# AdamBeedell/MLX8-WS-Audio-Transformer

Measured on AMD Instinct MI355X. Metric: 4s@16kHz clips/sec through mel+Whisper-small encoder, higher is better.
Workload: dtype fp16; 1 GPU; int16 PCM [B,64000] in HBM -> Whisper log-mel [B,80,3000] -> Whisper-small encoder -> hidden [B,1500,768] fp32; mode=parity (clip zero-padded to 30 s, as the reference computes), precision=f16f8, fp16_exact_projection_matrices=0 of 48 (found by the library at upload), parallelism=dp1 (clip shards, no data-path collective)

## Files before the change

### include/awt.h

```cpp
#ifndef AWT_H_
#define AWT_H_

#include <stddef.h>
#include <stdint.h>

#ifdef __cplusplus
extern "C" {
#endif

typedef enum awt_status {
  AWT_OK = 0,
  AWT_ERR_INVALID = -1,
  AWT_ERR_HIP = -2,
  AWT_ERR_WORKSPACE = -3,
  AWT_ERR_STATE = -4,
  AWT_ERR_VALUE = -5
} awt_status;

typedef struct awt_ctx awt_ctx;
typedef struct awt_encoder awt_encoder;

const char* awt_last_error(void);
const char* awt_version(void);

// ... 176 lines not shown
                            float* out, void* stream);
size_t awt_dtw_workspace_bytes(int clips, int T, int frames);
int awt_op_dtw(awt_ctx* c, const float* matrix, int clips, int T, int frames, const int32_t* num_frames, int negate, int32_t* jump_frame,
               int32_t* text_idx, int32_t* time_idx, int32_t* path_start, void* workspace, size_t ws_bytes, void* stream);

size_t awt_op_conv1d_workspace_bytes(int B, int T, int Cin, int Cout);
int awt_op_conv1d(awt_ctx* c, const float* x, const float* w, const float* bias, float* y, int B, int T, int Cin, int Cout, int taps, int terms,
                  void* workspace, size_t ws_bytes, void* stream);
size_t awt_op_batchnorm_stats_workspace_bytes(int M, int C);
int awt_op_batchnorm_stats(awt_ctx* c, const float* x, int M, int C, float* mean, float* var, void* workspace, size_t ws_bytes, void* stream);
enum { AWT_POOL_MEAN = 0, AWT_POOL_MAX2 = 2, AWT_POOL_MAX4 = 4, AWT_POOL_MAX4_MEAN = 5 };
int awt_op_bn_relu_pool(awt_ctx* c, const float* x, const float* mean, const float* var, const float* gamma, const float* beta, float eps,
                        float* y, int B, int T, int C, int pool, void* stream);
size_t awt_op_bn_relu_pool_backward_workspace_bytes(int B, int T, int C);
int awt_op_bn_relu_pool_backward(awt_ctx* c, const float* dy, const float* x, const float* mean, const float* var, const float* gamma,
                                 const float* beta, float eps, float* dx, float* dgamma, float* dbeta, int B, int T, int C, int pool,
                                 void* workspace, size_t ws_bytes, void* stream);

int awt_op_conv1d_framed(awt_ctx* c, const float* x, int64_t x_pitch, const float* w, const float* bias, float* y, int B, int n_samples, int kernel,
                         int stride, int Cout, void* stream);

int awt_tuning_set(const char* key, int value);

enum { AWT_PROF_LOGMEL = 0, AWT_PROF_GEMM = 1, AWT_PROF_ATTENTION = 2, AWT_PROF_LAYERNORM = 3, AWT_PROF_OTHER = 4,
       AWT_PROF_ATTENTION_BWD = 5,
       AWT_PROF_WGRAD = 6,
       AWT_PROF_NCLASSES = 7 };
int awt_prof_enable(awt_ctx* c, int mask);
int awt_prof_collect(awt_ctx* c, int klass, double* total_ms, int64_t* launches, double* flops);

#ifdef __cplusplus
}
#endif
#endif
```

### mlx8-ws-audio-transformer_amd/_lib.py

```python
from __future__ import annotations

import ctypes as C
import os
import re
import threading
from typing import Optional

import torch

HERE = os.path.dirname(os.path.abspath(__file__))
LIB_PATH = os.environ.get("AWT_LIB") or os.path.join(HERE, "libawt.so")
HEADER_PATH = os.path.join(os.path.dirname(HERE), "include", "awt.h")

AWT_OK = 0
AWT_ERR_VALUE = -5


class AwtError(RuntimeError):
    def __init__(self, code: int, msg: str):
        super().__init__(f"libawt error {code}: {msg}")
        self.code = code
        self.msg = msg


# ... 88 lines not shown
    "awt_op_attention_small": (_i, [_vp, _vp, _i, _vp, _i, _vp, _i, _vp, _i, _vp, _i, _i, _i, _i, _i, _i, _vp]),
    "awt_op_attention_small_backward": (_i, [_vp, _vp, _i, _vp, _i, _vp, _i, _vp, _vp, _i, _vp, _vp, _vp, _vp, _vp, _i, _i, _i, _i, _i, _i, _vp]),
    "awt_op_attention_small_dropout": (_i, [_vp, _vp, _i, _vp, _i, _vp, _i, _vp, _i, _vp, _i, _i, _i, _i, _i, _i, C.c_float, C.c_uint64, _vp]),
    "awt_op_attention_small_backward_dropout": (_i, [_vp, _vp, _i, _vp, _i, _vp, _i, _vp, _vp, _i, _vp, _vp, _vp, _vp, _vp, _i, _i, _i, _i, _i, _i, C.c_float, C.c_uint64, _vp]),
    "awt_op_attention_cached": (_i, [_vp, _vp, _i, _vp, _vp, _i, _i64, _vp, _i, _i, _i, _i, _i, _vp]),
    "awt_select_tokens_workspace_bytes": (_sz, [_i, _i, _i]),
    "awt_op_select_tokens": (_i, [_vp, _vp, _i, _i, _i, _i, _vp, _vp, _i, _i, _vp, _vp, _vp, _vp, _sz, _vp]),
    "awt_select_tokens_ts_workspace_bytes": (_sz, [_i, _i, _i]),
    "awt_op_select_tokens_ts": (_i, [_vp, _vp, _i, _i, _i, _i, _vp, _vp, _i, _i, _vp, _vp, _vp, _vp, _vp, _sz, _vp]),
    "awt_op_kv_gather": (_i, [_vp, _vp, _vp, _vp, _i, _i, _i, _i, _i, _i, _vp]),
    "awt_op_alignment_weights": (_i, [_vp, _vp, _i, _i, _i, _i, _i, _vp, _i, _i, _vp, _i, _vp, _i, _i, _i, _vp, _i, _vp]),
    "awt_op_alignment_matrix": (_i, [_vp, _vp, _i, _i, _i, _i, _vp, _i, _vp, _vp]),
    "awt_dtw_workspace_bytes": (_sz, [_i, _i, _i]),
    "awt_op_dtw": (_i, [_vp, _vp, _i, _i, _i, _vp, _i, _vp, _vp, _vp, _vp, _vp, _sz, _vp]),
    "awt_op_conv1d_workspace_bytes": (_sz, [_i, _i, _i, _i]),
    "awt_op_conv1d": (_i, [_vp, _vp, _vp, _vp, _vp, _i, _i, _i, _i, _i, _i, _vp, _sz, _vp]),
    "awt_op_batchnorm_stats_workspace_bytes": (_sz, [_i, _i]),
    "awt_op_batchnorm_stats": (_i, [_vp, _vp, _i, _i, _vp, _vp, _vp, _sz, _vp]),
    "awt_op_bn_relu_pool": (_i, [_vp, _vp, _vp, _vp, _vp, _vp, _f, _vp, _i, _i, _i, _i, _vp]),
    "awt_op_bn_relu_pool_backward_workspace_bytes": (_sz, [_i, _i, _i]),
    "awt_op_bn_relu_pool_backward": (_i, [_vp, _vp, _vp, _vp, _vp, _vp, _vp, _f, _vp, _vp, _vp, _i, _i, _i, _i, _vp, _sz, _vp]),
    "awt_op_conv1d_framed": (_i, [_vp, _vp, _i64, _vp, _vp, _vp, _i, _i, _i, _i, _i, _vp]),
    "awt_tuning_set": (_i, [C.c_char_p, _i]),
    "awt_prof_enable": (_i, [_vp, _i]),
    "awt_prof_collect": (_i, [_vp, _i, C.POINTER(C.c_double), C.POINTER(_i64), C.POINTER(C.c_double)]),
}

_lib = None
_lock = threading.Lock()
_ctx = {}


def declared_symbols() -> list:
    text = open(HEADER_PATH).read()
    text = re.sub(r"/\*.*?\*/", "", text, flags=re.S)
    return sorted(set(re.findall(r"\b(awt_[a-z0-9_]+)\s*\(", text)))


def lib() -> C.CDLL:
    global _lib
    with _lock:
        if _lib is None:
            if not os.path.exists(LIB_PATH):
                raise ImportError(f"{LIB_PATH} is missing: run `python -m mlx8_ws_audio_transformer_amd.build` "
                                  "(there is no CPU fallback for this path)")
            l = C.CDLL(LIB_PATH)
# ... 69 lines not shown
```

### mlx8-ws-audio-transformer_amd/csrc/awt_api.hip

```cpp
#include <string.h>
#include <algorithm>
#include <string>
#include <vector>

#include "common.h"
#include "comm.h"
#include "wgrad.h"

static thread_local std::string g_err;
void awt_set_error(const std::string& msg) { g_err = msg; }
int awt_fail(int code, const std::string& msg) { g_err = msg; return code; }
extern "C" const char* awt_last_error(void) { return g_err.c_str(); }
extern "C" const char* awt_version(void) { return "awt 0.1 (gfx950)"; }

struct awt_prof_state {
  struct Span { hipEvent_t a, b; };
  std::vector<Span> spans[AWT_PROF_NCLASSES];
  std::vector<Span> pool;
  double flops[AWT_PROF_NCLASSES] = {};
  Span open[AWT_PROF_NCLASSES];
};

void awt_prof_begin(awt_ctx* c, int klass, hipStream_t s, double flops) {
  awt_prof_state* p = c->prof;
// ... 14 lines not shown
static int g_pp_mask = 12;
extern "C" int awt_tuning_set(const char* key, int value) {
  AWT_REQUIRE(key, AWT_ERR_INVALID, "tuning_set: null key");
  if (!strcmp(key, "gemm_tile")) {
    AWT_REQUIRE(value == 0 || value == 64 || value == 128 || value == 256, AWT_ERR_INVALID, "tuning_set: gemm_tile must be 0 (auto), 64, 128 or 256");
    awt_gemm_force_tile(value);
    return AWT_OK;
  }
  if (!strcmp(key, "gemm_gm")) {
    AWT_REQUIRE(value >= 0 && value <= 64, AWT_ERR_INVALID, "tuning_set: gemm_gm must be 0 (default) .. 64");
    awt_gemm_set_gm(value);
    return AWT_OK;
  }
  if (!strcmp(key, "gemm_pp")) {
    AWT_REQUIRE(value >= 0 && value <= 2, AWT_ERR_INVALID, "tuning_set: gemm_pp must be 0 (off), 1 (automatic, default) or 2 (wherever supported)");
    awt_gemm_set_pp_mode(value);
    return AWT_OK;
  }
  if (!strcmp(key, "gemm_pp_mask")) {
    AWT_REQUIRE(value >= 0 && value <= 15, AWT_ERR_INVALID, "tuning_set: gemm_pp_mask is a bit set 0 .. 15 (1 qkv, 2 out_proj, 4 fc1, 8 fc2; fc2 only together with fc1)");
    g_pp_mask = value;
    return AWT_OK;
  }
  if (!strcmp(key, "gemm_mfma16")) {
    AWT_REQUIRE(value == 0 || value == 1, AWT_ERR_INVALID, "tuning_set: gemm_mfma16 must be 1 (default: the f16f8 GEMM's 16 x 16 MFMA form where it applies) or 0 (32 x 32 only)");
    awt_gemm_set_mfma16(value);
    return AWT_OK;
  }
  if (!strcmp(key, "conv_live")) {
    AWT_REQUIRE(value == 0 || value == 1, AWT_ERR_INVALID, "tuning_set: conv_live must be 1 (default: the conv stem of awt_audio_encode computes the live positions only) or 0 (every position)");
    g_conv_live = value;
    return AWT_OK;
  }
  if (!strcmp(key, "attn_shape")) {
    AWT_REQUIRE(value == 0 || (value >= 4 && value <= 6), AWT_ERR_INVALID, "tuning_set: attn_shape must be 0 (auto), 4, 5 or 6");
    awt_attn_force_shape(value);
    return AWT_OK;
  }
  if (!strcmp(key, "attn_qt")) {
    AWT_REQUIRE(value >= 0 && value <= 2, AWT_ERR_INVALID, "tuning_set: attn_qt must be 0 (auto), 1 or 2");
    awt_attn_force_qt(value);
    return AWT_OK;
  }
  AWT_REQUIRE(false, AWT_ERR_INVALID, "tuning_set: unknown key");
}

extern "C" int awt_prof_enable(awt_ctx* c, int on) {
  AWT_REQUIRE(c, AWT_ERR_INVALID, "prof_enable: null ctx");
  if (!c->prof) c->prof = new awt_prof_state();
  c->prof_on = on;
  return AWT_OK;
}
extern "C" int awt_prof_collect(awt_ctx* c, int klass, double* total_ms, int64_t* launches, double* flops) {
  AWT_REQUIRE(c && c->prof && klass >= 0 && klass < AWT_PROF_NCLASSES, AWT_ERR_INVALID, "prof_collect: bad argument");
  awt_prof_state* p = c->prof;
  double ms = 0;
  for (auto& sp : p->spans[klass]) {
    AWT_HIP_CHECK(hipEventSynchronize(sp.b));
    float t = 0;
    AWT_HIP_CHECK(hipEventElapsedTime(&t, sp.a, sp.b));
    ms += t;
    p->pool.push_back(sp);
  }
  if (total_ms) *total_ms = ms;
  if (launches) *launches = (int64_t)p->spans[klass].size();
  if (flops) *flops = p->flops[klass];
  p->spans[klass].clear();
  p->flops[klass] = 0;
// ... 1150 lines not shown
```

### mlx8-ws-audio-transformer_amd/csrc/common.h

```cpp
#pragma once
#include <hip/hip_runtime.h>
#include <stdint.h>
#include <string>

#include "../../include/awt.h"

typedef unsigned short bf16_t;
typedef short bf16x8 __attribute__((ext_vector_type(8)));
typedef short bf16x4 __attribute__((ext_vector_type(4)));
typedef float f32x4 __attribute__((ext_vector_type(4)));
typedef float f32x16 __attribute__((ext_vector_type(16)));
typedef double f64x4 __attribute__((ext_vector_type(4)));

typedef _Float16 f16x8 __attribute__((ext_vector_type(8)));
typedef int i32x8 __attribute__((ext_vector_type(8)));
typedef int i32x2 __attribute__((ext_vector_type(2)));

#define AWT_WAVE 64

enum { PREC_BF16 = 1, PREC_F16 = 2, PREC_BF16X3 = 3, PREC_F16X3 = 4, PREC_F16F8 = 5 };
__host__ __device__ constexpr bool prec_known(int p) { return p >= PREC_BF16 && p <= PREC_F16F8; }
__host__ __device__ constexpr bool prec_is_f16(int p) { return p == PREC_F16 || p == PREC_F16X3 || p == PREC_F16F8; }
__host__ __device__ constexpr int prec_products(int p) { return (p == PREC_BF16 || p == PREC_F16) ? 1 : 3; }
constexpr int kF8Act = -2;
// ... 292 lines not shown
  uint8_t* hi8; uint8_t* lo8;
  char* ilv;
  bf16_t* hi2; bf16_t* lo2;
  const bf16_t* pre_hi; const bf16_t* pre_lo;
  const float* bias;
  const float* pos; int rows_pos;
  float scale;
  int n_valid;
  int S, H;
  int64_t plane_stride;
  int skip_v8;
  int m_pick;
};

int launch_gemm(awt_ctx* c, int M, int N, const GemmSeg* segs, int nseg, int prec, GemmEpilogue epi, const GemmOut& out,
                hipStream_t s);
bool gemm_pp_supported(int M, int N, int K, int epi);
int gemm_pp_slots();
int launch_gemm_pp(awt_ctx* c, int M, int N, const GemmSeg& seg, GemmEpilogue epi, const GemmOut& out, hipStream_t s);
size_t gemm_pp_weight_bytes(int N, int K);
int launch_pack_weight_pp(awt_ctx* c, const float* src, int N, int K, int row_off, char* dst, hipStream_t s);
int awt_gemm_pp_mode();
void awt_gemm_set_pp_mode(int v);
void awt_gemm_set_mfma16(int v);

int launch_layernorm(awt_ctx* c, const float* x, const float* gamma, const float* beta, int M, int d, float eps,
                     float* out_f32, const Act& out, int prec, hipStream_t s);
int launch_attention(awt_ctx* c, const bf16_t* q_hi, const bf16_t* q_lo, const bf16_t* k_hi, const bf16_t* k_lo,
                     const bf16_t* v_hi, const bf16_t* v_lo, bf16_t* o_hi, bf16_t* o_lo, float* o_f32, float* lse, int B, int H,
                     int S, int terms, hipStream_t s);
int launch_split_f32(awt_ctx* c, const float* x, int64_t n, float scale, bf16_t* hi, bf16_t* lo, hipStream_t s);
struct F8Planes { bf16_t* p16; uint8_t* hi8; uint8_t* lo8; };
int launch_split_planes(awt_ctx* c, const float* x, int64_t n, float scale, int prec, int f8_exp, bf16_t* p16, bf16_t* lo16, uint8_t* hi8,
                        uint8_t* lo8, hipStream_t s, char* ilv = nullptr);
int launch_attention_f16f8(awt_ctx* c, const F8Planes& q, const F8Planes& k, const F8Planes& v, const F8Planes& o, float* o_f32,
                           float* lse, int B, int H, int S, hipStream_t s, char* o_ilv = nullptr);
int launch_pack_weight(awt_ctx* c, const float* src, int N, int C, int taps, int64_t ld, int row_off, int col_off, float scale,
                       bf16_t* hi, bf16_t* lo, uint8_t* lo8, int prec, hipStream_t s, int* inexact = nullptr,
                       bf16_t* s16 = nullptr, uint8_t* s8 = nullptr);
int launch_im2col_conv1(awt_ctx* c, const float* mel, int B, int C, int T_mel, int T, int K_dst, const Act& out, int prec, hipStream_t s);
int launch_expand_conv_rows(awt_ctx* c, const float* g, const float* pos, int B, int S, int Sc, int d, float* x, hipStream_t s);
int conv_stem_positions(int n_ctx, int max_valid);

int logmel_whisper_impl(awt_ctx* c, const void* pcm, int pcm_is_i16, int64_t pcm_stride, const int32_t* n_valid,
                        int max_valid, int B, int n_frames_out, int n_mels, float* out, void* workspace, size_t ws_bytes, hipStream_t s,
                        int n_signal = 0);
// ... 28 lines not shown
```

### mlx8-ws-audio-transformer_amd/csrc/gemm.hip

```cpp
#include <algorithm>
#include <type_traits>
#include "common.h"
#include "gemm_pp.h"

#ifndef AWT_GEMM_GM
#define AWT_GEMM_GM 8
#endif

namespace {

int g_gm = AWT_GEMM_GM;
constexpr int kMaxSeg = 3;
typedef int i32x4_t __attribute__((ext_vector_type(4)));

struct GemmArgs {
  int M, N, nseg, tiles_m, tiles_n;
  int gm;
  GemmSeg seg[kMaxSeg];
  GemmOut out;
  const bf16_t* zeros;
  int64_t bs_a, bs_w, bs_o;
};

struct Cfg64 { static constexpr int WM = 2, WN = 2, TM = 2, TN = 4; };
// ... 904 lines not shown
template <int EPI>
int launch_f8s(GemmArgs a, hipStream_t s) {
  return launch_tiles<gemm_f8s_kernel<EPI>>(a, 128, 256, 256, 2 * (128 * 64 * 2 + 2 * 128 * 64), s);
}

template <int EPI, class CFG>
int launch_f8(GemmArgs a, hipStream_t s) {
  constexpr int BM = CFG::WM * CFG::TM * 32, BN = CFG::WN * CFG::TN * 32, NT = CFG::WM * CFG::WN * 64;
  constexpr int lds = 2 * (BM * 64 * 2 + 2 * BM * 64);
  if (a.nseg == 1 && a.seg[0].w_exact16) return launch_tiles<gemm_f8_kernel<EPI, CFG, false, true>>(a, BM, BN, NT, lds, s);
  if (a.nseg == 1) return launch_tiles<gemm_f8_kernel<EPI, CFG, false>>(a, BM, BN, NT, lds, s);
  return launch_tiles<gemm_f8_kernel<EPI, CFG, true>>(a, BM, BN, NT, lds, s);
}

template <int EPI, bool ILV>
__global__ __launch_bounds__(512, 2) void gemm_pp_kernel(pp::Args g, GemmOut out) {
  extern __shared__ __attribute__((aligned(16))) char smem[];
  const int lane = threadIdx.x & 63;
  const int wave = __builtin_amdgcn_readfirstlane(threadIdx.x >> 6);
  const int wr = wave >> 2, wc = wave & 3, r16 = lane & 15, kq = lane >> 4;
  float* patch = reinterpret_cast<float*>(smem + pp::PATCH_BASE + wave * 8192);
  const int c8 = (lane & 7) * 8, r8 = lane >> 3;
  constexpr bool SIDE = EPI == EPI_F32_RESID;
  pp::kloop(g, smem, [&](int tm, int tn, pp::Acc& accs) {
    auto& acc = accs.t;
    const int m0 = tm * pp::BM, n0 = tn * pp::BN;
    const int em0 = m0 + wr * 128, en = n0 + wc * 64 + c8;
    float4 b0 = make_float4(0.f, 0.f, 0.f, 0.f), b1 = b0;
    if (out.bias && en < out.n_valid) { b0 = *reinterpret_cast<const float4*>(out.bias + en); b1 = *reinterpret_cast<const float4*>(out.bias + en + 4); }
    auto strips = [&](auto full_t) {
      constexpr bool FULL = decltype(full_t)::value;
      float4 side[4][2], side_next[4][2];
      auto load_sides = [&](float4 (&d)[4][2], int i) {
#pragma unroll
        for (int it = 0; it < 4; ++it) {
          d[it][0] = load_side4<EPI, FULL>(out, em0 + i * 32 + r8 + 8 * it, en, g.M);
          d[it][1] = load_side4<EPI, FULL>(out, em0 + i * 32 + r8 + 8 * it, en + 4, g.M);
        }
      };
      if constexpr (SIDE) load_sides(side, 0);
#pragma unroll
      for (int i = 0; i < 4; ++i) {
#pragma unroll
        for (int rt = 0; rt < 2; ++rt)
#pragma unroll
          for (int ct = 0; ct < 4; ++ct)
#pragma unroll
            for (int reg = 0; reg < 4; ++reg) {
              const int row = rt * 16 + 4 * kq + reg;
              patch[row * 64 + (((ct * 16 + r16 + 16 * kq) & 63) ^ ((reg & 1) << 2))] = acc[2 * i + rt][ct][reg];
            }
        __builtin_amdgcn_wave_barrier();
        asm volatile("s_waitcnt lgkmcnt(0)" ::: "memory");
        if constexpr (SIDE) { if (i + 1 < 4) load_sides(side_next, i + 1); }
#pragma unroll
        for (int it = 0; it < 4; ++it) {
          const int rl = r8 + 8 * it, sw = (rl & 1) << 2, rot = 16 * ((rl >> 2) & 3);
          const float4 v0 = *reinterpret_cast<const float4*>(patch + rl * 64 + (((c8 + rot) & 63) ^ sw)), v1 = *reinterpret_cast<const float4*>(patch + rl * 64 + (((c8 + 4 + rot) & 63) ^ sw));
          store_out8_f8<EPI, FULL, ILV>(out, em0 + i * 32 + rl, en, v0, v1, side[it][0], side[it][1], b0, b1, g.M);
        }
        if constexpr (SIDE) {
#pragma unroll
          for (int it = 0; it < 4; ++it) { side[it][0] = side_next[it][0]; side[it][1] = side_next[it][1]; }
        }
        __builtin_amdgcn_wave_barrier();
        asm volatile("s_waitcnt lgkmcnt(0)" ::: "memory");
      }
    };
    if (m0 + pp::BM <= g.M && n0 + pp::BN <= out.n_valid) strips(std::true_type{}); else strips(std::false_type{});
  });
}

template <int EPI, bool ILV>
int launch_pp(const pp::Args& a, const GemmOut& o, int grid, hipStream_t s) {
  return launch_kernel<gemm_pp_kernel<EPI, ILV>>(dim3(grid), dim3(pp::NT), pp::LDS_BYTES, s, a, o);
}

int g_force_tile = 0;

template <int TERMS, int BK, int EPI, class CFG, bool F16, bool WX, bool BATCH>
int launch_one(GemmArgs a, hipStream_t s, int batch) {
  using T = Tile<TERMS, BK, CFG, WX>;
  return launch_tiles<gemm_kernel<TERMS, BK, EPI, CFG, F16, WX, BATCH>>(a, T::BM, T::BN, T::THREADS, T::LDS_BYTES, s, batch);
}
template <int TERMS, int EPI, bool F16, bool WX = false, bool BATCH = false>
int launch_tile(int tile, GemmArgs a, hipStream_t s, int batch = 1) {
  constexpr int BK = TERMS == 1 ? 64 : 32;
  if (tile == 256) return launch_one<TERMS, BK, EPI, CfgW4, F16, WX, BATCH>(a, s, batch);
  if (tile == 128) return launch_one<TERMS, BK, EPI, Cfg128, F16, WX, BATCH>(a, s, batch);
  return launch_one<TERMS, 64, EPI, Cfg64, F16, WX, BATCH>(a, s, batch);
}

constexpr int kSlots = 512;
// ... 37 lines not shown
}

int launch_gemm_batched(awt_ctx* c, int batch, int M, int N, int K, const bf16_t* a_hi, const bf16_t* a_lo, int64_t lda, int64_t bs_a, const bf16_t* w_hi,
                        const bf16_t* w_lo, int64_t bs_w, float* out, const float* resid, int64_t ldo, int64_t bs_o, int n_valid, hipStream_t s) {
  AWT_REQUIRE(c && c->zeros && batch > 0 && batch <= 65535 && M > 0 && N > 0 && N % 128 == 0 && K > 0 && K % 64 == 0, AWT_ERR_INVALID,
              "gemm (batched): 1..65535 matrices, N % 128 == 0 and K % 64 == 0 required");
  AWT_REQUIRE(a_hi && a_lo && w_hi && w_lo && out && lda % 8 == 0 && lda >= K && ldo % 4 == 0 && n_valid > 0 && n_valid <= N && n_valid % 4 == 0 && ldo >= n_valid, AWT_ERR_INVALID,
              "gemm (batched): null plane, lda not a multiple of 8, or output columns / pitch not a multiple of 4");
  AWT_REQUIRE(bs_a % 8 == 0 && bs_w % 8 == 0 && bs_o % 4 == 0, AWT_ERR_INVALID, "gemm (batched): matrix strides must keep 16-byte alignment");
  GemmArgs a{};
  a.M = M; a.N = N; a.nseg = 1; a.zeros = (const bf16_t*)c->zeros;
  GemmSeg& sg = a.seg[0];
  sg.a_hi = a_hi; sg.a_lo = a_lo; sg.lda = lda; sg.w_hi = w_hi; sg.w_lo = w_lo; sg.w_ksteps = K / 32; sg.w_k0 = 0; sg.K = K;
  sg.rows_out = sg.rows_in = M; sg.row_mul = 1; sg.row_add = 0;
  a.out.f32 = out; a.out.resid = resid; a.out.ldo = ldo; a.out.n_valid = n_valid;
  a.bs_a = bs_a; a.bs_w = bs_w; a.bs_o = bs_o;
  ProfScope prof(c, AWT_PROF_GEMM, s, 2.0 * (double)batch * (double)M * (double)n_valid * (double)K);
  return resid ? launch_batched_epi<EPI_F32_RESID>(a, batch, s) : launch_batched_epi<EPI_F32>(a, batch, s);
}

int g_pp_mode = 1;
int awt_gemm_pp_mode() { return g_pp_mode; }
void awt_gemm_set_pp_mode(int v) { g_pp_mode = v; }
int gemm_pp_slots() {
  static int n_cu[64] = {};
  int dev = 0;
  if (hipGetDevice(&dev) != hipSuccess) return 0;
  if (!n_cu[dev & 63]) { hipDeviceProp_t p; if (hipGetDeviceProperties(&p, dev) != hipSuccess) return 0; n_cu[dev & 63] = p.multiProcessorCount > 0 ? p.multiProcessorCount : 256; }
  return n_cu[dev & 63];
}
bool gemm_pp_supported(int M, int N, int K, int epi) {
  return M > 0 && N > 0 && N % 256 == 0 && K >= 128 && K % 64 == 0 &&
         (epi == EPI_F32 || epi == EPI_F32_RESID || epi == EPI_BF16 || epi == EPI_BF16_GELU || epi == EPI_QKV);
}
int launch_gemm_pp(awt_ctx* c, int M, int N, const GemmSeg& seg, GemmEpilogue epi, const GemmOut& out, hipStream_t s) {
  AWT_REQUIRE(c && gemm_pp_supported(M, N, seg.K, epi), AWT_ERR_INVALID, "gemm (ping-pong): N % 256 == 0, K % 64 == 0, K >= 128 and a supported epilogue required");
  AWT_REQUIRE(seg.a_ilv && seg.w_pp && seg.rows_out == M && seg.rows_in == M && seg.row_mul == 1 && seg.row_add == 0 && seg.w_k0 == 0 && seg.w_ksteps == seg.K / 32 && seg.lda == seg.K,
              AWT_ERR_INVALID, "gemm (ping-pong): one plain, dense K segment over split-line activations and a packed weight image");
  AWT_REQUIRE(!out.ilv || ((epi == EPI_BF16 || epi == EPI_BF16_GELU) && out.ldo == N && out.n_valid == N), AWT_ERR_INVALID, "gemm (ping-pong): a split-line output is a dense [M, N] activation");
  pp::Args a{};
  a.A = seg.a_ilv; a.a_row_bytes = (int64_t)seg.lda * 4; a.W = seg.w_pp;
  a.M = M; a.N = N; a.K = seg.K; a.nk = seg.K / 32;
  a.tiles_m = (M + pp::BM - 1) / pp::BM; a.tiles_n = N / pp::BN; a.ntiles = a.tiles_m * a.tiles_n; a.gm = g_gm;
  const int grid = std::min(a.ntiles, gemm_pp_slots());
  ProfScope prof(c, AWT_PROF_GEMM, s, 2.0 * (double)M * (double)out.n_valid * (double)seg.K);
  switch (epi) {
    case EPI_F32: return launch_pp<EPI_F32, false>(a, out, grid, s);
    case EPI_F32_RESID: return launch_pp<EPI_F32_RESID, false>(a, out, grid, s);
    case EPI_BF16: return out.ilv ? launch_pp<EPI_BF16, true>(a, out, grid, s) : launch_pp<EPI_BF16, false>(a, out, grid, s);
    case EPI_BF16_GELU: return out.ilv ? launch_pp<EPI_BF16_GELU, true>(a, out, grid, s) : launch_pp<EPI_BF16_GELU, false>(a, out, grid, s);
    case EPI_QKV: return launch_pp<EPI_QKV, false>(a, out, grid, s);
    default: break;
  }
  return awt_fail(AWT_ERR_INVALID, "gemm (ping-pong): unsupported epilogue");
}

void awt_gemm_set_mfma16(int v) { g_mfma16 = v; }
void awt_gemm_force_tile(int t) { g_force_tile = t; }
void awt_gemm_set_gm(int v) { g_gm = v > 0 ? v : AWT_GEMM_GM; }

int launch_gemm(awt_ctx* c, int M, int N, const GemmSeg* segs, int nseg, int prec, GemmEpilogue epi, const GemmOut& out,
                hipStream_t s) {
  AWT_REQUIRE(M > 0 && N > 0 && N % 128 == 0, AWT_ERR_INVALID, "gemm: N must be a positive multiple of 128");
  AWT_REQUIRE(nseg >= 1 && nseg <= kMaxSeg, AWT_ERR_INVALID, "gemm: 1..3 K-segments");
  AWT_REQUIRE(prec_known(prec), AWT_ERR_INVALID, "gemm: unknown operand precision");
  const int terms = prec_products(prec);
  AWT_REQUIRE(c && c->zeros, AWT_ERR_INVALID, "gemm: context without a zero page");
// ... 29 lines not shown
```

### mlx8-ws-audio-transformer_amd/csrc/gemm_pp.h

```cpp
#pragma once
#include <type_traits>
#include <utility>
#include "common.h"

namespace pp {

constexpr int BM = 256, BN = 256, NT = 512;
constexpr int REGION = 16384, BUF = 65536;
constexpr int OFF_A0 = 0, OFF_B0 = 16384, OFF_B1 = 32768, OFF_A1 = 49152;
constexpr int PATCH_BASE = BUF + OFF_B1;
constexpr int LDS_BYTES = PATCH_BASE + 8 * 8192;
struct Acc { f32x4 t[8][4]; };

__host__ __device__ __forceinline__ int64_t w_region_offset(int bn, int kt, int s, int nk) { return (((int64_t)bn * nk + kt) * 2 + s) * REGION; }
__host__ __device__ __forceinline__ int w_row_offset(int n_in_tile, int chunk) {
  const int rho = (n_in_tile >> 6) * 32 + (n_in_tile & 31);
  return rho * 128 + ((chunk ^ ((rho >> 1) & 7)) << 4);
}

struct Args {
  const char* A;
  int64_t a_row_bytes;
  const char* W;
  int M, N, K, nk;
  int tiles_m, tiles_n, ntiles, gm;
};

template <int OFF>
__device__ __forceinline__ bf16x8 dsr(unsigned addr) {
  bf16x8 v;
  asm volatile("ds_read_b128 %0, %1 offset:%2" : "=v"(v) : "v"(addr), "n"(OFF));
  return v;
}
__device__ __forceinline__ void dma_v(const char* src, unsigned lds_dst_uniform) {
  unsigned keep;
  asm volatile("s_mov_b32 %0, m0\n\ts_mov_b32 m0, %2\n\ts_nop 0\n\tglobal_load_lds_dwordx4 %1, off\n\ts_mov_b32 m0, %0"
               : "=&s"(keep) : "v"(src), "s"(lds_dst_uniform) : "memory");
}
__device__ __forceinline__ void dma_s(const char* sbase, unsigned voff, unsigned lds_dst_uniform) {
  unsigned keep;
  asm volatile("s_mov_b32 %0, m0\n\ts_mov_b32 m0, %3\n\ts_nop 0\n\tglobal_load_lds_dwordx4 %1, %2\n\ts_mov_b32 m0, %0"
               : "=&s"(keep) : "v"(voff), "s"(sbase), "s"(lds_dst_uniform) : "memory");
}
template <int N, class F> __device__ __forceinline__ void static_for(F&& f) {
  [&]<int... I>(std::integer_sequence<int, I...>) { (f(std::integral_constant<int, I>{}), ...); }(std::make_integer_sequence<int, N>{});
}
template <int N> __device__ __forceinline__ void vmwait() { asm volatile("s_waitcnt vmcnt(%0)" ::"n"(N) : "memory"); }

struct FragA { bf16x8 v[2][4]; };
struct FragB { bf16x8 v[4]; };

__device__ __forceinline__ void tie(FragA& a) {
  asm volatile("" : "+v"(a.v[0][0]), "+v"(a.v[0][1]), "+v"(a.v[0][2]), "+v"(a.v[0][3]), "+v"(a.v[1][0]), "+v"(a.v[1][1]), "+v"(a.v[1][2]), "+v"(a.v[1][3]));
}
__device__ __forceinline__ void tie(FragB& b) { asm volatile("" : "+v"(b.v[0]), "+v"(b.v[1]), "+v"(b.v[2]), "+v"(b.v[3])); }
__device__ __forceinline__ void lgkm0() { asm volatile("s_waitcnt lgkmcnt(0)" ::: "memory"); }

__device__ __forceinline__ i32x8 cat8(bf16x8 lo, bf16x8 hi) {
  typedef int i32x4_t __attribute__((ext_vector_type(4)));
  return __builtin_shufflevector(__builtin_bit_cast(i32x4_t, lo), __builtin_bit_cast(i32x4_t, hi), 0, 1, 2, 3, 4, 5, 6, 7);
}

__device__ __forceinline__ void mfma_y(f32x4& c, bf16x8 a0, bf16x8 a1, bf16x8 b0, bf16x8 b1) {
  c = __builtin_amdgcn_mfma_scale_f32_16x16x128_f8f6f4(cat8(a0, a1), cat8(b0, b1), c, 0, 0, 0, e8m0(-kF8Act), 0, e8m0(-kF8Wgt - kF8Lo));
}

template <class EPI>
__device__ __forceinline__ void kloop(const Args& g, char* smem, EPI&& epi) {
  const int lane = threadIdx.x & 63;
  const int wave = __builtin_amdgcn_readfirstlane(threadIdx.x >> 6);
  const int wr = wave >> 2, wc = wave & 3;
  const unsigned lds0 = (unsigned)(uintptr_t)(__attribute__((address_space(3))) char*)smem;
  const int nk = g.nk;
  const int nmine = (g.ntiles - (int)blockIdx.x + (int)gridDim.x - 1) / (int)gridDim.x;
  if (nmine <= 0) return;

  auto tile_coords = [&](int it, int& tm, int& tn) {
    gemm_tile_coords(xcd_contiguous((int)(blockIdx.x + it * gridDim.x), g.ntiles), g.tiles_m, g.tiles_n, g.gm, tm, tn);
  };

  constexpr int PIECES = 2;
  const char* ab[2];
  const char* wb[2];
  unsigned aoff[2];
#pragma unroll
  for (int e = 0; e < 2; ++e) {
    const int rho = (wave * PIECES + e) * 8 + (lane >> 3), c = (lane & 7) ^ ((rho >> 1) & 7);
    aoff[e] = (unsigned)(((rho >> 6) * 128 + (rho & 63) - 8 * e) * g.a_row_bytes + c * 16);
  }
  const unsigned wvoff = lane * 16;
  auto a_base = [&](int tm, int s) { return g.A + ((int64_t)tm * BM + s * 64) * g.a_row_bytes; };
  auto w_base = [&](int tn, int s) { return g.W + w_region_offset(tn, 0, s, nk); };
  auto stage_a = [&](auto s_t, auto buf_t) {
    constexpr int s = decltype(s_t)::value, buf = decltype(buf_t)::value;
    if (wave >= 0) {
      const unsigned dst = __builtin_amdgcn_readfirstlane(lds0 + buf * BUF + (s ? OFF_A1 : OFF_A0) + wave * PIECES * 1024);
#pragma unroll
      for (int i = 0; i < PIECES; ++i) dma_s(ab[s] + (int64_t)(8 * i) * g.a_row_bytes, aoff[i], dst + i * 1024);
    }
    ab[s] += 128;
  };
  auto stage_b = [&](auto s_t, auto buf_t) {
    constexpr int s = decltype(s_t)::value, buf = decltype(buf_t)::value;
    if (wave >= 0) {
      const unsigned dst = __builtin_amdgcn_readfirstlane(lds0 + buf * BUF + (s ? OFF_B1 : OFF_B0) + wave * PIECES * 1024);
#pragma unroll
      for (int i = 0; i < PIECES; ++i) dma_s(wb[s] + (wave * PIECES + i) * 1024, wvoff, dst + i * 1024);
    }
    wb[s] += 2 * REGION;
  };
  auto vmw = [&](auto n_t) { vmwait<decltype(n_t)::value * PIECES>(); };
  using R5 = std::integral_constant<int, 5>; using R4 = std::integral_constant<int, 4>;
  using I0 = std::integral_constant<int, 0>; using I1 = std::integral_constant<int, 1>;

  unsigned aaddr[4], baddr[4];
#pragma unroll
  for (int x = 0; x < 4; ++x) {
    const int r16 = lane & 15, f16 = (r16 >> 1) & 7, kq = lane >> 4, chunk = x < 2 ? 4 * x + kq : 2 * kq + (x - 2);
    aaddr[x] = lds0 + (x < 2 ? 0 : BUF) + (wr * 64 + r16) * 128 + ((chunk ^ f16) << 4);
    baddr[x] = lds0 + (x < 2 ? 0 : BUF) + (wc * 32 + r16) * 128 + ((chunk ^ f16) << 4);
  }
  auto read_a = [&](auto s_t, FragA& a, auto par_t) {
    constexpr int base = decltype(s_t)::value ? OFF_A1 : OFF_A0, par = decltype(par_t)::value;
    static_for<4>([&](auto x_t) {
      constexpr int x = decltype(x_t)::value, ai = 2 * par + (x & 1);
      a.v[0][x] = dsr<base + (x >> 1) * 2048>(aaddr[ai]); a.v[1][x] = dsr<base + 4096 + (x >> 1) * 2048>(aaddr[ai]);
    });
  };
  auto read_b = [&](auto s_t, FragB& b, auto par_t) {
    constexpr int base = decltype(s_t)::value ? OFF_B1 : OFF_B0, par = decltype(par_t)::value;
    static_for<4>([&](auto x_t) {
      constexpr int x = decltype(x_t)::value;
      b.v[x] = dsr<base + (x >> 1) * 2048>(baddr[2 * par + (x & 1)]);
    });
  };

  Acc accs;
  auto& acc = accs.t;
  auto zero_acc = [&]() {
#pragma unroll
    for (int i = 0; i < 8; ++i)
#pragma unroll
      for (int j = 0; j < 4; ++j) acc[i][j] = (f32x4){};
  };
  auto mma = [&](auto sa_t, auto sb_t, const FragA& a, const FragB& b, auto par_t) {
    constexpr int sa = decltype(sa_t)::value, sb = decltype(sb_t)::value, par = decltype(par_t)::value;
    __builtin_amdgcn_sched_barrier(0);
    __builtin_amdgcn_s_setprio(1);
    if constexpr (par == 1) {
#pragma unroll
      for (int rt = 0; rt < 4; ++rt)
#pragma unroll
        for (int ct = 0; ct < 2; ++ct)
          mfma_y(acc[4 * sa + rt][2 * sb + ct], a.v[rt >> 1][(rt & 1) * 2], a.v[rt >> 1][(rt & 1) * 2 + 1], b.v[ct * 2], b.v[ct * 2 + 1]);
    } else {
#pragma unroll
      for (int ks = 0; ks < 2; ++ks)
#pragma unroll
        for (int rt = 0; rt < 4; ++rt)
#pragma unroll
          for (int ct = 0; ct < 2; ++ct)
            acc[4 * sa + rt][2 * sb + ct] = mfma16<true>(a.v[rt >> 1][(rt & 1) * 2 + ks], b.v[ct * 2 + ks], acc[4 * sa + rt][2 * sb + ct]);
    }
#pragma unroll
    for (int rt = 0; rt < 4; ++rt) asm volatile("" : "+v"(acc[4 * sa + rt][2 * sb]), "+v"(acc[4 * sa + rt][2 * sb + 1]));
    __builtin_amdgcn_s_setprio(0);
    __builtin_amdgcn_sched_barrier(0);
  };
  auto bar = [&]() { __builtin_amdgcn_s_barrier(); };

  int tm, tn, tm1, tn1;
  tile_coords(0, tm, tn);
  tile_coords(nmine > 1 ? 1 : 0, tm1, tn1);
  ab[0] = a_base(tm, 0); ab[1] = a_base(tm, 1); wb[0] = w_base(tn, 0); wb[1] = w_base(tn, 1);

  stage_b(I0{}, I0{}); stage_a(I0{}, I0{}); stage_b(I1{}, I0{}); stage_a(I1{}, I0{});
  stage_b(I0{}, I1{}); stage_a(I0{}, I1{});
  vmw(R4{});
  bar();

  FragA ra; FragB rba, rbb;
  auto pair = [&](auto last_t) {
    constexpr bool LAST = decltype(last_t)::value;
    read_a(I0{}, ra, I0{}); stage_a(I1{}, I1{}); vmw(R5{}); bar();
    lgkm0(); tie(ra); tie(rba); mma(I0{}, I0{}, ra, rba, I0{}); bar();
    if constexpr (LAST) wb[0] = w_base(tn1, 0);
    read_b(I1{}, rbb, I0{}); stage_b(I0{}, I0{}); vmw(R5{}); bar();
    lgkm0(); tie(rbb); mma(I0{}, I1{}, ra, rbb, I0{}); bar();
    if constexpr (LAST) ab[0] = a_base(tm1, 0);
    read_a(I1{}, ra, I0{}); stage_a(I0{}, I0{}); vmw(R5{}); bar();
    lgkm0(); tie(ra); mma(I1{}, I1{}, ra, rbb, I0{}); bar();
    if constexpr (LAST) wb[1] = w_base(tn1, 1);
    read_b(I0{}, rbb, I1{}); stage_b(I1{}, I0{}); vmw(R4{}); bar();
    mma(I1{}, I0{}, ra, rba, I0{}); bar();
    if constexpr (LAST) ab[1] = a_base(tm1, 1);
    read_a(I0{}, ra, I1{}); stage_a(I1{}, I0{}); vmw(R5{}); bar();
    lgkm0(); tie(ra); tie(rbb); mma(I0{}, I0{}, ra, rbb, I1{}); bar();
    read_b(I1{}, rba, I1{}); stage_b(I0{}, I1{}); vmw(R5{}); bar();
    lgkm0(); tie(rba); mma(I0{}, I1{}, ra, rba, I1{}); bar();
    read_a(I1{}, ra, I1{}); stage_a(I0{}, I1{}); vmw(R5{}); bar();
    lgkm0(); tie(ra); mma(I1{}, I1{}, ra, rba, I1{}); bar();
    if constexpr (!LAST) { read_b(I0{}, rba, I0{}); stage_b(I1{}, I1{}); }
    vmw(R4{}); bar();
    mma(I1{}, I0{}, ra, rbb, I1{}); bar();
  };

  for (int it = 0; it < nmine; ++it) {
    zero_acc();
    if (wr == 1) bar();
    read_b(I0{}, rba, I0{});
    stage_b(I1{}, I1{});
    for (int kp = 2; kp < nk; kp += 2) pair(std::false_type{});
    pair(std::true_type{});
    if (wr == 0) bar();
    epi(tm, tn, accs);
    tm = tm1; tn = tn1;
    tile_coords(it + 2 < nmine ? it + 2 : nmine - 1, tm1, tn1);
    lgkm0();
    bar();
  }
  vmwait<0>();
}

}
```

Measured before the change: 1423 clips/s.

## Split partly filled last GEMM round into half-height tiles for ping-pong kernel

Adds a tail-balancing rule to the ping-pong f16f8 GEMM. When the tile count leaves a partly filled final wave of workgroups, the last M panels are recomputed as 128-row tiles, which doubles the tile count in that region. A cost model chooses whether to split, with half tiles assumed to cost a fraction rho of a full tile. The kloop is templated on tile height, with adjusted wait counts, fragment sizes and workgroup offsets so half tiles fill the slots left idle by the full tiles. This targets idle CUs in the last round, at the price of a second kloop instantiation, more code and less reuse in the half tiles.

After: 1434 clips/s, median of 6. About the same (+0.8%).

```diff
diff --git a/include/awt.h b/include/awt.h
--- a/include/awt.h
+++ b/include/awt.h
@@ -222,6 +222,9 @@
 
 int awt_tuning_set(const char* key, int value);
 
+int awt_gemm_pp_tail_panels(int tiles_m, int tiles_n, int workgroups, int K, int mode);
+double awt_gemm_pp_tail_rho(int K);
+
 enum { AWT_PROF_LOGMEL = 0, AWT_PROF_GEMM = 1, AWT_PROF_ATTENTION = 2, AWT_PROF_LAYERNORM = 3, AWT_PROF_OTHER = 4,
        AWT_PROF_ATTENTION_BWD = 5,
        AWT_PROF_WGRAD = 6,
diff --git a/mlx8-ws-audio-transformer_amd/_lib.py b/mlx8-ws-audio-transformer_amd/_lib.py
--- a/mlx8-ws-audio-transformer_amd/_lib.py
+++ b/mlx8-ws-audio-transformer_amd/_lib.py
@@ -134,6 +134,8 @@
     "awt_op_bn_relu_pool_backward": (_i, [_vp, _vp, _vp, _vp, _vp, _vp, _vp, _f, _vp, _vp, _vp, _i, _i, _i, _i, _vp, _sz, _vp]),
     "awt_op_conv1d_framed": (_i, [_vp, _vp, _i64, _vp, _vp, _vp, _i, _i, _i, _i, _i, _vp]),
     "awt_tuning_set": (_i, [C.c_char_p, _i]),
+    "awt_gemm_pp_tail_panels": (_i, [_i, _i, _i, _i, _i]),
+    "awt_gemm_pp_tail_rho": (C.c_double, [_i]),
     "awt_prof_enable": (_i, [_vp, _i]),
     "awt_prof_collect": (_i, [_vp, _i, C.POINTER(C.c_double), C.POINTER(_i64), C.POINTER(C.c_double)]),
 }
diff --git a/mlx8-ws-audio-transformer_amd/csrc/awt_api.hip b/mlx8-ws-audio-transformer_amd/csrc/awt_api.hip
--- a/mlx8-ws-audio-transformer_amd/csrc/awt_api.hip
+++ b/mlx8-ws-audio-transformer_amd/csrc/awt_api.hip
@@ -60,6 +60,16 @@
     g_pp_mask = value;
     return AWT_OK;
   }
+  if (!strcmp(key, "gemm_pp_tail")) {
+    AWT_REQUIRE(value >= 0 && value <= 2, AWT_ERR_INVALID, "tuning_set: gemm_pp_tail must be 0 (off), 1 (by the split rule, default) or 2 (every partly filled last round)");
+    awt_gemm_set_pp_tail_mode(value);
+    return AWT_OK;
+  }
+  if (!strcmp(key, "gemm_pp_wgs")) {
+    AWT_REQUIRE(value >= 0 && value <= 1024, AWT_ERR_INVALID, "tuning_set: gemm_pp_wgs must be 0 (one workgroup per CU, default) .. 1024");
+    awt_gemm_set_pp_wgs(value);
+    return AWT_OK;
+  }
   if (!strcmp(key, "gemm_mfma16")) {
     AWT_REQUIRE(value == 0 || value == 1, AWT_ERR_INVALID, "tuning_set: gemm_mfma16 must be 1 (default: the f16f8 GEMM's 16 x 16 MFMA form where it applies) or 0 (32 x 32 only)");
     awt_gemm_set_mfma16(value);
@@ -82,6 +92,11 @@
   }
   AWT_REQUIRE(false, AWT_ERR_INVALID, "tuning_set: unknown key");
 }
+
+extern "C" int awt_gemm_pp_tail_panels(int tiles_m, int tiles_n, int workgroups, int K, int mode) {
+  return gemm_pp_tail_panels(tiles_m, tiles_n, workgroups, gemm_pp_rho(K), mode);
+}
+extern "C" double awt_gemm_pp_tail_rho(int K) { return gemm_pp_rho(K); }
 
 extern "C" int awt_prof_enable(awt_ctx* c, int on) {
   AWT_REQUIRE(c, AWT_ERR_INVALID, "prof_enable: null ctx");
diff --git a/mlx8-ws-audio-transformer_amd/csrc/common.h b/mlx8-ws-audio-transformer_amd/csrc/common.h
--- a/mlx8-ws-audio-transformer_amd/csrc/common.h
+++ b/mlx8-ws-audio-transformer_amd/csrc/common.h
@@ -338,6 +338,11 @@
 int launch_pack_weight_pp(awt_ctx* c, const float* src, int N, int K, int row_off, char* dst, hipStream_t s);
 int awt_gemm_pp_mode();
 void awt_gemm_set_pp_mode(int v);
+int awt_gemm_pp_tail_mode();
+void awt_gemm_set_pp_tail_mode(int v);
+void awt_gemm_set_pp_wgs(int v);
+double gemm_pp_rho(int K);
+int gemm_pp_tail_panels(int tiles_m, int tiles_n, int wgs, double rho, int mode);
 void awt_gemm_set_mfma16(int v);
 
 int launch_layernorm(awt_ctx* c, const float* x, const float* gamma, const float* beta, int M, int d, float eps,
diff --git a/mlx8-ws-audio-transformer_amd/csrc/gemm.hip b/mlx8-ws-audio-transformer_amd/csrc/gemm.hip
--- a/mlx8-ws-audio-transformer_amd/csrc/gemm.hip
+++ b/mlx8-ws-audio-transformer_amd/csrc/gemm.hip
@@ -950,10 +950,11 @@
   float* patch = reinterpret_cast<float*>(smem + pp::PATCH_BASE + wave * 8192);
   const int c8 = (lane & 7) * 8, r8 = lane >> 3;
   constexpr bool SIDE = EPI == EPI_F32_RESID;
-  pp::kloop(g, smem, [&](int tm, int tn, pp::Acc& accs) {
+  auto epi = [&](auto h_t, int row0, int tm, int tn, auto& accs) {
+    constexpr int H = decltype(h_t)::value;
     auto& acc = accs.t;
-    const int m0 = tm * pp::BM, n0 = tn * pp::BN;
-    const int em0 = m0 + wr * 128, en = n0 + wc * 64 + c8;
+    const int m0 = row0 + tm * H, n0 = tn * pp::BN;
+    const int em0 = m0 + wr * (H / 2), en = n0 + wc * 64 + c8;
     float4 b0 = make_float4(0.f, 0.f, 0.f, 0.f), b1 = b0;
     if (out.bias && en < out.n_valid) { b0 = *reinterpret_cast<const float4*>(out.bias + en); b1 = *reinterpret_cast<const float4*>(out.bias + en + 4); }
     auto strips = [&](auto full_t) {
@@ -968,7 +969,7 @@
       };
       if constexpr (SIDE) load_sides(side, 0);
 #pragma unroll
-      for (int i = 0; i < 4; ++i) {
+      for (int i = 0; i < H / 64; ++i) {
 #pragma unroll
         for (int rt = 0; rt < 2; ++rt)
 #pragma unroll
@@ -980,7 +981,7 @@
             }
         __builtin_amdgcn_wave_barrier();
         asm volatile("s_waitcnt lgkmcnt(0)" ::: "memory");
-        if constexpr (SIDE) { if (i + 1 < 4) load_sides(side_next, i + 1); }
+        if constexpr (SIDE) { if (i + 1 < H / 64) load_sides(side_next, i + 1); }
 #pragma unroll
         for (int it = 0; it < 4; ++it) {
           const int rl = r8 + 8 * it, sw = (rl & 1) << 2, rot = 16 * ((rl >> 2) & 3);
@@ -995,8 +996,10 @@
         asm volatile("s_waitcnt lgkmcnt(0)" ::: "memory");
       }
     };
-    if (m0 + pp::BM <= g.M && n0 + pp::BN <= out.n_valid) strips(std::true_type{}); else strips(std::false_type{});
-  });
+    if (m0 + H <= g.M && n0 + pp::BN <= out.n_valid) strips(std::true_type{}); else strips(std::false_type{});
+  };
+  pp::kloop<256>(g, smem, [&](int tm, int tn, pp::AccT<256>& accs) { epi(std::integral_constant<int, 256>{}, 0, tm, tn, accs); });
+  if (g.half_m > 0) pp::kloop<128>(g, smem, [&](int tm, int tn, pp::AccT<128>& accs) { epi(std::integral_constant<int, 128>{}, g.tiles_m * pp::BM, tm, tn, accs); });
 }
 
 template <int EPI, bool ILV>
@@ -1080,12 +1083,28 @@
 int g_pp_mode = 1;
 int awt_gemm_pp_mode() { return g_pp_mode; }
 void awt_gemm_set_pp_mode(int v) { g_pp_mode = v; }
+int g_pp_tail = 1, g_pp_wgs = 0;
+int awt_gemm_pp_tail_mode() { return g_pp_tail; }
+void awt_gemm_set_pp_tail_mode(int v) { g_pp_tail = v; }
+void awt_gemm_set_pp_wgs(int v) { g_pp_wgs = v; }
 int gemm_pp_slots() {
+  if (g_pp_wgs > 0) return g_pp_wgs;
   static int n_cu[64] = {};
   int dev = 0;
   if (hipGetDevice(&dev) != hipSuccess) return 0;
   if (!n_cu[dev & 63]) { hipDeviceProp_t p; if (hipGetDeviceProperties(&p, dev) != hipSuccess) return 0; n_cu[dev & 63] = p.multiProcessorCount > 0 ? p.multiProcessorCount : 256; }
   return n_cu[dev & 63];
+}
+constexpr double kPpRhoK768 = 0.52, kPpRhoK3072 = 0.57;
+double gemm_pp_rho(int K) { return K < (768 + 3072) / 2 ? kPpRhoK768 : kPpRhoK3072; }
+int gemm_pp_tail_panels(int tiles_m, int tiles_n, int wgs, double rho, int mode) {
+  if (mode == 0 || tiles_m <= 0 || tiles_n <= 0 || wgs <= 0) return 0;
+  const int64_t t = (int64_t)tiles_m * tiles_n, r = t % wgs;
+  if (r == 0) return 0;
+  const int64_t h = (r + tiles_n - 1) / tiles_n, full = t - h * tiles_n, halves = 2 * h * tiles_n;
+  if (mode == 2) return (int)h;
+  const double split = (double)((full + wgs - 1) / wgs) + (double)((halves + wgs - 1) / wgs) * rho, whole = (double)((t + wgs - 1) / wgs);
+  return split < whole ? (int)h : 0;
 }
 bool gemm_pp_supported(int M, int N, int K, int epi) {
   return M > 0 && N > 0 && N % 256 == 0 && K >= 128 && K % 64 == 0 &&
@@ -1099,8 +1118,13 @@
   pp::Args a{};
   a.A = seg.a_ilv; a.a_row_bytes = (int64_t)seg.lda * 4; a.W = seg.w_pp;
   a.M = M; a.N = N; a.K = seg.K; a.nk = seg.K / 32;
-  a.tiles_m = (M + pp::BM - 1) / pp::BM; a.tiles_n = N / pp::BN; a.ntiles = a.tiles_m * a.tiles_n; a.gm = g_gm;
-  const int grid = std::min(a.ntiles, gemm_pp_slots());
+  const int panels = (M + pp::BM - 1) / pp::BM, slots = gemm_pp_slots();
+  AWT_REQUIRE(slots > 0, AWT_ERR_HIP, "gemm (ping-pong): no device");
+  a.tiles_n = N / pp::BN; a.gm = g_gm;
+  a.tiles_m = panels - gemm_pp_tail_panels(panels, a.tiles_n, slots, gemm_pp_rho(seg.K), g_pp_tail);
+  a.ntiles = a.tiles_m * a.tiles_n;
+  a.half_m = a.tiles_m < panels ? (M - a.tiles_m * pp::BM + 127) / 128 : 0;
+  const int grid = std::min(a.ntiles + a.half_m * a.tiles_n, slots);
   ProfScope prof(c, AWT_PROF_GEMM, s, 2.0 * (double)M * (double)out.n_valid * (double)seg.K);
   switch (epi) {
     case EPI_F32: return launch_pp<EPI_F32, false>(a, out, grid, s);
diff --git a/mlx8-ws-audio-transformer_amd/csrc/gemm_pp.h b/mlx8-ws-audio-transformer_amd/csrc/gemm_pp.h
--- a/mlx8-ws-audio-transformer_amd/csrc/gemm_pp.h
+++ b/mlx8-ws-audio-transformer_amd/csrc/gemm_pp.h
@@ -10,7 +10,8 @@
 constexpr int OFF_A0 = 0, OFF_B0 = 16384, OFF_B1 = 32768, OFF_A1 = 49152;
 constexpr int PATCH_BASE = BUF + OFF_B1;
 constexpr int LDS_BYTES = PATCH_BASE + 8 * 8192;
-struct Acc { f32x4 t[8][4]; };
+template <int H> struct AccT { f32x4 t[H / 32][4]; };
+using Acc = AccT<BM>;
 
 __host__ __device__ __forceinline__ int64_t w_region_offset(int bn, int kt, int s, int nk) { return (((int64_t)bn * nk + kt) * 2 + s) * REGION; }
 __host__ __device__ __forceinline__ int w_row_offset(int n_in_tile, int chunk) {
@@ -24,6 +25,7 @@
   const char* W;
   int M, N, K, nk;
   int tiles_m, tiles_n, ntiles, gm;
+  int half_m;
 };
 
 template <int OFF>
@@ -47,12 +49,13 @@
 }
 template <int N> __device__ __forceinline__ void vmwait() { asm volatile("s_waitcnt vmcnt(%0)" ::"n"(N) : "memory"); }
 
-struct FragA { bf16x8 v[2][4]; };
+template <int H> struct FragAT { bf16x8 v[H / 128][4]; };
 struct FragB { bf16x8 v[4]; };
 
-__device__ __forceinline__ void tie(FragA& a) {
+__device__ __forceinline__ void tie(FragAT<256>& a) {
   asm volatile("" : "+v"(a.v[0][0]), "+v"(a.v[0][1]), "+v"(a.v[0][2]), "+v"(a.v[0][3]), "+v"(a.v[1][0]), "+v"(a.v[1][1]), "+v"(a.v[1][2]), "+v"(a.v[1][3]));
 }
+__device__ __forceinline__ void tie(FragAT<128>& a) { asm volatile("" : "+v"(a.v[0][0]), "+v"(a.v[0][1]), "+v"(a.v[0][2]), "+v"(a.v[0][3])); }
 __device__ __forceinline__ void tie(FragB& b) { asm volatile("" : "+v"(b.v[0]), "+v"(b.v[1]), "+v"(b.v[2]), "+v"(b.v[3])); }
 __device__ __forceinline__ void lgkm0() { asm volatile("s_waitcnt lgkmcnt(0)" ::: "memory"); }
 
@@ -65,38 +68,54 @@
   c = __builtin_amdgcn_mfma_scale_f32_16x16x128_f8f6f4(cat8(a0, a1), cat8(b0, b1), c, 0, 0, 0, e8m0(-kF8Act), 0, e8m0(-kF8Wgt - kF8Lo));
 }
 
-template <class EPI>
+constexpr int pieces_a(int h) { return h / 128; }
+constexpr int kPiecesB = 2;
+constexpr int wait_pieces(int h, int phase) {
+  return phase == 2 ? 2 * pieces_a(h) + 3 * kPiecesB : phase == 4 ? 2 * pieces_a(h) + 2 * kPiecesB : 3 * pieces_a(h) + 2 * kPiecesB;
+}
+static_assert(wait_pieces(256, 1) == 10 && wait_pieces(256, 2) == 10 && wait_pieces(256, 3) == 10 && wait_pieces(256, 4) == 8, "height 256: five / four regions x two pieces");
+static_assert(wait_pieces(128, 1) == 7 && wait_pieces(128, 2) == 8 && wait_pieces(128, 3) == 7 && wait_pieces(128, 4) == 6, "height 128: A regions are one piece per wave");
+
+template <int H = BM, class EPI>
 __device__ __forceinline__ void kloop(const Args& g, char* smem, EPI&& epi) {
+  static_assert(H == 256 || H == 128, "tile height");
+  constexpr bool HALF = H == 128;
+  constexpr int RT = H / 64;
   const int lane = threadIdx.x & 63;
   const int wave = __builtin_amdgcn_readfirstlane(threadIdx.x >> 6);
   const int wr = wave >> 2, wc = wave & 3;
   const unsigned lds0 = (unsigned)(uintptr_t)(__attribute__((address_space(3))) char*)smem;
   const int nk = g.nk;
-  const int nmine = (g.ntiles - (int)blockIdx.x + (int)gridDim.x - 1) / (int)gridDim.x;
+  const int tiles_m = HALF ? g.half_m : g.tiles_m, ntiles = HALF ? g.half_m * g.tiles_n : g.ntiles;
+  int wg = (int)blockIdx.x;
+  if constexpr (HALF) { wg -= g.ntiles % (int)gridDim.x; if (wg < 0) wg += (int)gridDim.x; }
+  const int nmine = (ntiles - wg + (int)gridDim.x - 1) / (int)gridDim.x;
   if (nmine <= 0) return;
 
   auto tile_coords = [&](int it, int& tm, int& tn) {
-    gemm_tile_coords(xcd_contiguous((int)(blockIdx.x + it * gridDim.x), g.ntiles), g.tiles_m, g.tiles_n, g.gm, tm, tn);
-  };
-
-  constexpr int PIECES = 2;
+    gemm_tile_coords(xcd_contiguous((int)(wg + it * gridDim.x), ntiles), tiles_m, g.tiles_n, g.gm, tm, tn);
+  };
+
+  constexpr int PIECES_A = pieces_a(H), PIECES = kPiecesB;
   const char* ab[2];
   const char* wb[2];
-  unsigned aoff[2];
-#pragma unroll
-  for (int e = 0; e < 2; ++e) {
-    const int rho = (wave * PIECES + e) * 8 + (lane >> 3), c = (lane & 7) ^ ((rho >> 1) & 7);
-    aoff[e] = (unsigned)(((rho >> 6) * 128 + (rho & 63) - 8 * e) * g.a_row_bytes + c * 16);
+  unsigned aoff[PIECES_A];
+#pragma unroll
+  for (int e = 0; e < PIECES_A; ++e) {
+    const int rho = (wave * PIECES_A + e) * 8 + (lane >> 3), c = (lane & 7) ^ ((rho >> 1) & 7);
+    const int row = HALF ? (rho >> 5) * 64 + (rho & 31) : (rho >> 6) * 128 + (rho & 63);
+    aoff[e] = (unsigned)((row - 8 * e) * g.a_row_bytes + c * 16);
   }
   const unsigned wvoff = lane * 16;
-  auto a_base = [&](int tm, int s) { return g.A + ((int64_t)tm * BM + s * 64) * g.a_row_bytes; };
+  const int64_t row0 = HALF ? (int64_t)g.tiles_m * BM : 0;
+  auto a_base = [&](int tm, int s) { return g.A + (row0 + (int64_t)tm * H + s * (H / 4)) * g.a_row_bytes; };
   auto w_base = [&](int tn, int s) { return g.W + w_region_offset(tn, 0, s, nk); };
   auto stage_a = [&](auto s_t, auto buf_t) {
     constexpr int s = decltype(s_t)::value, buf = decltype(buf_t)::value;
     if (wave >= 0) {
-      const unsigned dst = __builtin_amdgcn_readfirstlane(lds0 + buf * BUF + (s ? OFF_A1 : OFF_A0) + wave * PIECES * 1024);
-#pragma unroll
-      for (int i = 0; i < PIECES; ++i) dma_s(ab[s] + (int64_t)(8 * i) * g.a_row_bytes, aoff[i], dst + i * 1024);
+      const unsigned dst = __builtin_amdgcn_readfirstlane(lds0 + buf * BUF + (s ? OFF_A1 : OFF_A0) + wave * PIECES_A * 1024);
+#pragma unroll
+      for (int i = 0; i < PIECES_A; ++i) dma_s(ab[s] + (int64_t)(8 * i) * g.a_row_bytes, aoff[i], dst + i * 1024);
     }
     ab[s] += 128;
   };
@@ -109,22 +128,24 @@
     }
     wb[s] += 2 * REGION;
   };
-  auto vmw = [&](auto n_t) { vmwait<decltype(n_t)::value * PIECES>(); };
-  using R5 = std::integral_constant<int, 5>; using R4 = std::integral_constant<int, 4>;
+  auto vmw = [&](auto ph_t) { vmwait<wait_pieces(H, decltype(ph_t)::value)>(); };
+  using W1 = std::integral_constant<int, 1>; using W2 = std::integral_constant<int, 2>; using W3 = std::integral_constant<int, 3>; using W4 = std::integral_constant<int, 4>;
   using I0 = std::integral_constant<int, 0>; using I1 = std::integral_constant<int, 1>;
 
   unsigned aaddr[4], baddr[4];
 #pragma unroll
   for (int x = 0; x < 4; ++x) {
     const int r16 = lane & 15, f16 = (r16 >> 1) & 7, kq = lane >> 4, chunk = x < 2 ? 4 * x + kq : 2 * kq + (x - 2);
-    aaddr[x] = lds0 + (x < 2 ? 0 : BUF) + (wr * 64 + r16) * 128 + ((chunk ^ f16) << 4);
+    aaddr[x] = lds0 + (x < 2 ? 0 : BUF) + (wr * (H / 4) + r16) * 128 + ((chunk ^ f16) << 4);
     baddr[x] = lds0 + (x < 2 ? 0 : BUF) + (wc * 32 + r16) * 128 + ((chunk ^ f16) << 4);
   }
+  using FragA = FragAT<H>;
   auto read_a = [&](auto s_t, FragA& a, auto par_t) {
     constexpr int base = decltype(s_t)::value ? OFF_A1 : OFF_A0, par = decltype(par_t)::value;
     static_for<4>([&](auto x_t) {
       constexpr int x = decltype(x_t)::value, ai = 2 * par + (x & 1);
-      a.v[0][x] = dsr<base + (x >> 1) * 2048>(aaddr[ai]); a.v[1][x] = dsr<base + 4096 + (x >> 1) * 2048>(aaddr[ai]);
+      a.v[0][x] = dsr<base + (x >> 1) * 2048>(aaddr[ai]);
+      if constexpr (!HALF) a.v[1][x] = dsr<base + 4096 + (x >> 1) * 2048>(aaddr[ai]);
     });
   };
   auto read_b = [&](auto s_t, FragB& b, auto par_t) {
@@ -135,11 +156,11 @@
     });
   };
 
-  Acc accs;
+  AccT<H> accs;
   auto& acc = accs.t;
   auto zero_acc = [&]() {
 #pragma unroll
-    for (int i = 0; i < 8; ++i)
+    for (int i = 0; i < 2 * RT; ++i)
 #pragma unroll
       for (int j = 0; j < 4; ++j) acc[i][j] = (f32x4){};
   };
@@ -149,21 +170,21 @@
     __builtin_amdgcn_s_setprio(1);
     if constexpr (par == 1) {
 #pragma unroll
-      for (int rt = 0; rt < 4; ++rt)
+      for (int rt = 0; rt < RT; ++rt)
 #pragma unroll
         for (int ct = 0; ct < 2; ++ct)
-          mfma_y(acc[4 * sa + rt][2 * sb + ct], a.v[rt >> 1][(rt & 1) * 2], a.v[rt >> 1][(rt & 1) * 2 + 1], b.v[ct * 2], b.v[ct * 2 + 1]);
+          mfma_y(acc[RT * sa + rt][2 * sb + ct], a.v[rt >> 1][(rt & 1) * 2], a.v[rt >> 1][(rt & 1) * 2 + 1], b.v[ct * 2], b.v[ct * 2 + 1]);
     } else {
 #pragma unroll
       for (int ks = 0; ks < 2; ++ks)
 #pragma unroll
-        for (int rt = 0; rt < 4; ++rt)
+        for (int rt = 0; rt < RT; ++rt)
 #pragma unroll
           for (int ct = 0; ct < 2; ++ct)
-            acc[4 * sa + rt][2 * sb + ct] = mfma16<true>(a.v[rt >> 1][(rt & 1) * 2 + ks], b.v[ct * 2 + ks], acc[4 * sa + rt][2 * sb + ct]);
+            acc[RT * sa + rt][2 * sb + ct] = mfma16<true>(a.v[rt >> 1][(rt & 1) * 2 + ks], b.v[ct * 2 + ks], acc[RT * sa + rt][2 * sb + ct]);
     }
 #pragma unroll
-    for (int rt = 0; rt < 4; ++rt) asm volatile("" : "+v"(acc[4 * sa + rt][2 * sb]), "+v"(acc[4 * sa + rt][2 * sb + 1]));
+    for (int rt = 0; rt < RT; ++rt) asm volatile("" : "+v"(acc[RT * sa + rt][2 * sb]), "+v"(acc[RT * sa + rt][2 * sb + 1]));
     __builtin_amdgcn_s_setprio(0);
     __builtin_amdgcn_sched_barrier(0);
   };
@@ -176,32 +197,32 @@
 
   stage_b(I0{}, I0{}); stage_a(I0{}, I0{}); stage_b(I1{}, I0{}); stage_a(I1{}, I0{});
   stage_b(I0{}, I1{}); stage_a(I0{}, I1{});
-  vmw(R4{});
+  vmw(W4{});
   bar();
 
   FragA ra; FragB rba, rbb;
   auto pair = [&](auto last_t) {
     constexpr bool LAST = decltype(last_t)::value;
-    read_a(I0{}, ra, I0{}); stage_a(I1{}, I1{}); vmw(R5{}); bar();
+    read_a(I0{}, ra, I0{}); stage_a(I1{}, I1{}); vmw(W1{}); bar();
     lgkm0(); tie(ra); tie(rba); mma(I0{}, I0{}, ra, rba, I0{}); bar();
     if constexpr (LAST) wb[0] = w_base(tn1, 0);
-    read_b(I1{}, rbb, I0{}); stage_b(I0{}, I0{}); vmw(R5{}); bar();
+    read_b(I1{}, rbb, I0{}); stage_b(I0{}, I0{}); vmw(W2{}); bar();
     lgkm0(); tie(rbb); mma(I0{}, I1{}, ra, rbb, I0{}); bar();
     if constexpr (LAST) ab[0] = a_base(tm1, 0);
-    read_a(I1{}, ra, I0{}); stage_a(I0{}, I0{}); vmw(R5{}); bar();
+    read_a(I1{}, ra, I0{}); stage_a(I0{}, I0{}); vmw(W3{}); bar();
     lgkm0(); tie(ra); mma(I1{}, I1{}, ra, rbb, I0{}); bar();
     if constexpr (LAST) wb[1] = w_base(tn1, 1);
-    read_b(I0{}, rbb, I1{}); stage_b(I1{}, I0{}); vmw(R4{}); bar();
+    read_b(I0{}, rbb, I1{}); stage_b(I1{}, I0{}); vmw(W4{}); bar();
     mma(I1{}, I0{}, ra, rba, I0{}); bar();
     if constexpr (LAST) ab[1] = a_base(tm1, 1);
-    read_a(I0{}, ra, I1{}); stage_a(I1{}, I0{}); vmw(R5{}); bar();
+    read_a(I0{}, ra, I1{}); stage_a(I1{}, I0{}); vmw(W1{}); bar();
     lgkm0(); tie(ra); tie(rbb); mma(I0{}, I0{}, ra, rbb, I1{}); bar();
-    read_b(I1{}, rba, I1{}); stage_b(I0{}, I1{}); vmw(R5{}); bar();
+    read_b(I1{}, rba, I1{}); stage_b(I0{}, I1{}); vmw(W2{}); bar();
     lgkm0(); tie(rba); mma(I0{}, I1{}, ra, rba, I1{}); bar();
-    read_a(I1{}, ra, I1{}); stage_a(I0{}, I1{}); vmw(R5{}); bar();
+    read_a(I1{}, ra, I1{}); stage_a(I0{}, I1{}); vmw(W3{}); bar();
     lgkm0(); tie(ra); mma(I1{}, I1{}, ra, rba, I1{}); bar();
     if constexpr (!LAST) { read_b(I0{}, rba, I0{}); stage_b(I1{}, I1{}); }
-    vmw(R4{}); bar();
+    vmw(W4{}); bar();
     mma(I1{}, I0{}, ra, rbb, I1{}); bar();
   };
 
```
